# rwdavies/QUILT

Hardware: AMD Instinct MI355X
Metric: samples/sec on 2Mb region, K=50k haps, 1x coverage; dosage r2 vs CPU ref (higher is better)
Workload: dtype f64

## Files before the change

### quilt_amd/csrc/fullpass.hip

```cpp
#include "fullpass_dev.hpp"
#include "fullpass_testhook.h"
#include "pass_layout.hpp"

#include <algorithm>
#include <chrono>
#include <cmath>
#include <functional>
#include <memory>
#include <utility>

namespace {

template <typename TS>
__global__ __launch_bounds__(256) void k_emat(PassParams prm) {
    const int g = blockIdx.x, p = blockIdx.y, t = threadIdx.x;
    __shared__ double2 s_e[32];
    __shared__ double s_red[3][4];
    __shared__ int s_var;
    const int s = 32 * g;
    const int nLocal = min(32, prm.T - s);
    const double2 *gl = reinterpret_cast<const double2 *>(prm.gl) + (size_t)p * prm.T + s;
    if (t == 0) s_var = 0;
    __syncthreads();
    if (t < nLocal) {
// ... 638 lines not shown
    const int32_t *er = p.ent_read + p.ent_off[s], *eb = p.ent_bq + p.ent_off[s];
    const int32_t *H = p.H + p.pass_hoff[pi];
    double a = 1.0, b = 1.0;
    for (int i = sp[t]; i < sp[t + 1]; i++) {
        const int bq = eb[i];
        if (bq == 0 || H[er[i]] != lab) continue;
        const int ab = bq < 0 ? -bq : bq;
        a *= p.pR_tab[(bq > 0 ? 256 : 0) + ab];
        b *= p.pA_tab[(bq > 0 ? 256 : 0) + ab];
    }
    if (p.minGLValue > 0 && (a < p.minGLValue || b < p.minGLValue)) {
        if (a > b) { b = b / a; a = 1; if (b < p.minGLValue) b = p.minGLValue; }
        else       { a = a / b; b = 1; if (a < p.minGLValue) a = p.minGLValue; }
    }
    double2 *out = reinterpret_cast<double2 *>(p.gl) + (size_t)pi * p.T + t;
    *out = make_double2(a, b);
}

template <typename TS>
__global__ void k_unpermute(const TS *src, double *dst, int K, int Kq, int NT, int cols, size_t dst_ld) {
    constexpr int EPV = Vec<TS>::EPV, NV = 16 / EPV;
    const int col = blockIdx.y;
    const int k = blockIdx.x * blockDim.x + threadIdx.x;
    if (k >= K || col >= cols) return;
    const int chunk = k >> 4, e = k & 15;
    const int j = chunk / NT, t = chunk % NT;
    const size_t vec = alpha_vec_index<NV>(j, e / EPV, NT, t);
    dst[(size_t)col * dst_ld + k] = (double)src[(size_t)col * Kq + vec * EPV + (e % EPV)];
}

}

struct qa_panel::Scratch {
    qa::ABuf<double> gl, c, dosage, escale0, unperm, emin, emin_b1, spill, fw_add, fw_xs, gamma_col;
    qa::ABuf<char> emat, esp, alpha, gamma, beta, beta_thin, top_val, mg, gsp;
    qa::ABuf<int32_t> thin_col, flags, alpha_slot, top_cnt, top_idx;
    qa::DBuf<int32_t> todo;
    hipEvent_t ev[6] = {nullptr, nullptr, nullptr, nullptr, nullptr, nullptr};
    explicit Scratch(qa::Arena *a) {
        gl.arena = c.arena = dosage.arena = escale0.arena = unperm.arena = emin.arena = emin_b1.arena = spill.arena = fw_add.arena = fw_xs.arena = a;
        gamma_col.arena = a;
        emat.arena = esp.arena = alpha.arena = mg.arena = gsp.arena = gamma.arena = beta.arena = beta_thin.arena = top_val.arena = a;
        thin_col.arena = flags.arena = alpha_slot.arena = top_cnt.arena = top_idx.arena = a;
    }
    ~Scratch() {
        for (auto &e : ev) if (e) (void)hipEventDestroy(e);
    }
};

void qa::drop_pass_scratch(qa_panel *p) {
    delete p->scratch;
    p->scratch = nullptr;
}

qa_panel::~qa_panel() {
    delete scratch;
    if (gibbs_stream) (void)hipStreamDestroy(gibbs_stream);
    if (pass_stream) (void)hipStreamDestroy(pass_stream);
    if (stream) (void)hipStreamDestroy(stream);
}

namespace {

thread_local double g_timing[6] = {0, 0, 0, 0, 0, 0};

using qa::PassKind; using qa::KIND_F32; using qa::KIND_F64_RANK; using qa::KIND_F64_FULL; using qa::KIND_F64_DOS; using qa::KIND_F64_REF;
using qa::Geometry; using qa::PanelDims; using qa::PassLayout; using qa::Thin;
static_assert(qa::kLayoutMaxRow == kMaxRow, "pass_layout.hpp sizes emat / mg rows of kMaxRow");

struct KindInfo { const char *name; int pk_fwd, pk_bwd; };
constexpr KindInfo kKindInfo[qa::KIND_COUNT] = {
     {"fp32", qa::PK_FWD, qa::PK_BWD},
     {"fp64 ranking", qa::PK_FWD64, qa::PK_BWD64},
     {"generic fp64", qa::PK_FWD64G, qa::PK_BWD64G},
     {"fp64 dosage", qa::PK_FWD64D, qa::PK_BWD64D},
     {"reference-order validation", qa::PK_FWD64G, qa::PK_BWD64G},
};

constexpr int kNchList32[] = {1, 2, 3, 4, 5, 6, 7, 8, 10, 12};
constexpr int kNchList64[] = {1, 2, 4, 6, 8, 10, 12, 13, 14};
Geometry pick_geometry(int K, PassKind kind = KIND_F32) {
    const int chunks = (K + 15) / 16;
    if (kind == KIND_F64_RANK || kind == KIND_F64_DOS) {
        int nch = qa::fb64_chunks(K);
        if (kind == KIND_F64_DOS && nch && qa::fb64_dos_lds_bytes(K) > 160 * 1024) nch = 0;
        return {nch ? 512 : 0, nch, kind};
    }
    if (kind == KIND_F64_FULL || kind == KIND_F64_REF) {
        const int need = (K + 4095) / 4096;
        for (int nch : kNchList64) if (nch >= need) return {256, nch, kind};
        return {0, 0, kind};
    }
    auto fit = [&](int nch) -> int {
        int nt = (chunks + nch - 1) / nch;
        nt = std::max((nt + 63) / 64 * 64, 64);
        if (nt > 512) return 0;
        if (nch == 1 && chunks > 128) return 0;
        return nt;
    };
    for (int nch : kNchList32) if (int nt = fit(nch)) return {nt, nch, kind};
    return {0, 0, kind};
}


struct LastPlan { int64_t P = 0, per_pass = 0, fixed = 0, carved = 0, kind = 0; };
thread_local LastPlan g_last_plan;

PanelDims dims_of(const qa_panel *pn) { return {pn->K, pn->G, pn->T, pn->n_special, pn->n_sp_grids}; }

size_t plan_pass_bytes(const qa_panel *pn, const Geometry &geo, int32_t flag, const Thin &thin, int K_top, int top_cap = 64,
                       bool gamma_col = false) {
    return PassLayout(dims_of(pn), geo, qa::make_request(&flag, 1, thin, K_top, top_cap, gamma_col)).pass_bytes(qa::Arena::kCarveAlign);
}

int plan_chunk(qa_panel *pn, size_t per_pass, int remaining, size_t extra_fixed = 0) {
    const size_t fixed = (size_t)pn->G * 8 + ((size_t)2 << 20) + extra_fixed;
    g_last_plan.per_pass = (int64_t)per_pass;
    g_last_plan.fixed = (int64_t)fixed;
    const size_t budget = pn->plan_budget();
    long n = budget > fixed ? (long)((budget - fixed) / per_pass) : 0;
    n = std::max<long>(1, std::min<long>(n, remaining));
    static const int n_cu = [] {
        int dev = 0;
        hipDeviceProp_t prop;
        if (hipGetDevice(&dev) != hipSuccess || hipGetDeviceProperties(&prop, dev) != hipSuccess) return 256;
        return std::max(prop.multiProcessorCount, 1);
    }();
    if (n < remaining && n > n_cu) n = n / n_cu * n_cu;
    pn->require_scratch(fixed + (size_t)n * per_pass);
    pn->A().reset();
    return (int)n;
}

template <typename TS, int NCH, int MAXT, bool FULL>
void launch_fb(const PassParams &prm, int NT, hipStream_t s, hipEvent_t e_mid) {
    const size_t lds_f = 2 * kMaxRow * sizeof(TS) + 2 * 16 * 8;
    const size_t lds_b = lds_f + (FULL ? (size_t)2 * kMaxRow * kHistCopies * sizeof(typename Vec<TS>::Hist) : 0);
    hipLaunchKernelGGL((k_fwd<TS, NCH, MAXT>), dim3(prm.P), dim3(NT), lds_f, s, prm);
    QA_HIP(hipGetLastError());
// ... 142 lines not shown
std::vector<int32_t> plan_alpha_slots(const PassRun &r) {
    const int P = r.P, G = r.pn->G;
    std::vector<int32_t> slot((size_t)P * G, -1);
    for (int p = 0; p < P; p++) {
        int32_t *sl = slot.data() + (size_t)p * G;
        if ((r.h_flags[p] & 15) && r.geo.kind == KIND_F64_DOS) {
            for (int g = 0; g < G; g += 2) sl[g] = g / 2;
        } else if (r.h_flags[p] & 15) {
            for (int g = 0; g < G; g++) sl[g] = g;
        } else {
            int n = 0;
            for (int g = 0; g < G; g++) if (r.thin_col_h[g] >= 0) sl[g] = n++;
        }
    }
    return slot;
}

template <typename T>
void carve(qa::ABuf<T> &buf, const PassLayout &L, PassLayout::Buf b, int P) { buf.ensure(L.bytes(b, P) / sizeof(T)); }

void carve_scratch(qa_panel::Scratch &S, const PassLayout &L, int P, bool gl) {
    using B = PassLayout;
    if (gl) carve(S.gl, L, B::GL, P);
    carve(S.thin_col, L, B::THIN_COL, P);
    carve(S.flags, L, B::FLAGS, P);
    carve(S.alpha_slot, L, B::ALPHA_SLOT, P);
    carve(S.emat, L, B::EMAT, P);
    carve(S.escale0, L, B::ESCALE0, P);
    carve(S.emin, L, B::EMIN, P);
    carve(S.emin_b1, L, B::EMIN_B1, P);
    carve(S.esp, L, B::ESP, P);
    carve(S.gsp, L, B::GSP, P);
    carve(S.alpha, L, B::ALPHA, P);
    carve(S.c, L, B::C, P);
    carve(S.fw_add, L, B::FW_ADD, P);
    carve(S.fw_xs, L, B::FW_XS, P);
    carve(S.mg, L, B::MG, P);
    carve(S.dosage, L, B::DOSAGE, P);
    carve(S.gamma, L, B::GAMMA, P);
    carve(S.beta, L, B::BETA, P);
    carve(S.beta_thin, L, B::BETA_THIN, P);
    carve(S.gamma_col, L, B::GAMMA_COL, P);
    carve(S.top_cnt, L, B::TOP_CNT, P);
    carve(S.spill, L, B::SPILL, P);
    carve(S.top_idx, L, B::TOP_IDX, P);
    carve(S.top_val, L, B::TOP_VAL, P);
}

void fill_params(PassRun &r, int K_top, int normalize_emissions, int always_normalize, double norm_threshold) {
    const qa_panel *pn = r.pn;
    const auto &S = r.S;
    const PassLayout &L = r.L;
    const PassKind kind = r.geo.kind;
    PassParams &prm = r.prm;
    prm = PassParams{};
    prm.hm = pn->hm.p; prm.B = pn->B.p; prm.sp_off = pn->sp_off.p; prm.sp_k = pn->sp_k.p;
    prm.sp_word = pn->sp_word.p; prm.sp_gidx = pn->sp_gidx.p; prm.sp_chunk_at = pn->sp_chunk_at.p;
    prm.sigma = pn->sigma.p; prm.tm1 = pn->tm1.p; prm.IE = pn->ie_derived ? nullptr : pn->IE.p;
    prm.K = pn->K; prm.Kp = pn->Kp; prm.G = pn->G; prm.T = pn->T; prm.nMaxDH = pn->nMaxDH; prm.nrow = pn->nrow;
    prm.n_special = pn->n_special; prm.ref_error = pn->ref_error;
    prm.P = r.P; prm.gl = S.gl.p; prm.thin_col = S.thin_col.p; prm.n_thin = r.n_thin; prm.flags = S.flags.p;
    prm.normalize_emissions = normalize_emissions;
    prm.lazy = qa::lazy_kind(kind) ? 1 : 0; prm.always_normalize = always_normalize; prm.norm_threshold = norm_threshold;
    prm.grid0_left_to_right = pn->sum_order_grid0_ltr ? 1 : 0;
    prm.emin = S.emin.p; prm.emin_b1 = S.emin_b1.p; prm.esp_stride = (int)L.esp_stride;

    prm.spill = S.spill.p; prm.spill_pass_stride = L.spill_stride;
    prm.fw_add = S.fw_add.p; prm.fw_xs = S.fw_xs.p;
    prm.emat = S.emat.p; prm.esp = S.esp.p; prm.escale0 = S.escale0.p; prm.alpha = S.alpha.p; prm.alpha_slot = S.alpha_slot.p;
    prm.alpha_pass_stride = L.alpha_cols * L.alpha_col_elems; prm.Kq = (int)L.Kq; prm.alpha_col_elems = L.alpha_col_elems;
    prm.hist_unit = kind == KIND_F64_DOS ? 1.0 / 2251799813685248.0  : 1.0 / kHistScale64; prm.c = S.c.p; prm.mg = S.mg.p; prm.gsp = S.gsp.p;
    prm.gamma_out = S.gamma.p; prm.beta_out = S.beta.p;
    prm.gamma_col = S.gamma_col.p; prm.gamma_grid = r.out.gamma_col ? r.out.gamma_grid : -1;
    prm.K_top = r.any_top ? K_top : 0;
    prm.beta_thin = S.beta_thin.p;
    prm.fused_topk = r.fused ? 1 : 0;
    prm.top_cap = r.top_cap;
    prm.truncate_lists = r.out.truncate_lists ? 1 : 0;
    if (r.any_top) { prm.top_cnt = S.top_cnt.p; prm.top_idx = S.top_idx.p; prm.top_val = S.top_val.p; }
}

void choose_dosage_destination(PassRun &r) {
    const BatchOut &out = r.out;
    const int P = r.P, T = r.pn->T;
    bool direct = false;
    if (out.dosage && P > 0) {
        const size_t r0 = out.dosage_rows ? (size_t)out.dosage_rows[0] : 0;
        direct = true;
        for (int p = 0; p < P && direct; p++)
            direct = (r.h_flags[p] & 1) && (out.dosage_rows ? (size_t)out.dosage_rows[p] : (size_t)p) == r0 + (size_t)p;
        direct = direct && qa::pinned_registry().covers(out.dosage + r0 * T, sizeof(double) * (size_t)P * T);
        if (direct) r.prm.dosage = out.dosage + r0 * T;
    }
    if (!direct) r.prm.dosage = r.S.dosage.p;
    r.dosage_direct = direct;
}

void launch_passes(PassRun &r) {
    auto &S = r.S;
    const PassParams &prm = r.prm;
    const int P = r.P, G = r.pn->G;
// ... 294 lines not shown
    if (!out) return QA_ERR_INVALID;
    for (int i = 0; i < 3; i++) out[i] = g_timing[i];
    out[3] = g_timing[3] + g_timing[4];
    out[4] = g_timing[5];
    return QA_OK;
}

static int pack_lists(const std::vector<std::vector<std::pair<int32_t, double>>> &lists, int32_t *best_ptr,
                      int32_t *best_idx, double *best_val, int64_t best_cap) {
    if (!best_ptr) return QA_OK;
    int64_t total = 0;
    best_ptr[0] = 0;
    for (size_t i = 0; i < lists.size(); i++) {
        total += (int64_t)lists[i].size();
        best_ptr[i + 1] = (int32_t)total;
    }
    if (total > best_cap || !best_idx || !best_val) {
        qa::set_error("best-haps capacity %lld < needed %lld", (long long)best_cap, (long long)total);
        return QA_ERR_CAPACITY;
    }
    for (size_t i = 0; i < lists.size(); i++)
        for (size_t q = 0; q < lists[i].size(); q++) {
            best_idx[best_ptr[i] + q] = lists[i][q].first;
            best_val[best_ptr[i] + q] = (double)lists[i][q].second;
        }
    return QA_OK;
}

int qa_fullpass_last_plan(int64_t out[6]) {
    if (!out) return QA_ERR_INVALID;
    out[0] = g_last_plan.P; out[1] = g_last_plan.per_pass; out[2] = g_last_plan.fixed; out[3] = g_last_plan.carved;
    out[4] = PassLayout::N_BUF; out[5] = g_last_plan.kind;
    return QA_OK;
}

int qa_fullpass_launch_set(qa_panel_t *panel, int32_t n_pass, const double *gl, const int32_t *flags,
                           const int32_t *gammaSmall_cols_to_get, int32_t K_top_matches, int32_t always_normalize,
                           double *dosage, double *c, int32_t *best_ptr, int32_t *best_idx, double *best_val, int64_t best_cap) {
    if (!qa::device_ready()) return QA_ERR_NO_DEVICE;
    if (!panel || !gl || n_pass <= 0 || !flags || !gammaSmall_cols_to_get) {
        qa::set_error("qa_fullpass_launch_set: bad argument");
        return QA_ERR_INVALID;
    }
    int32_t any = 0;
    for (int i = 0; i < n_pass; i++) {
        if (flags[i] != 0 && flags[i] != 1) {
            qa::set_error("qa_fullpass_launch_set: flags must be 0 or 1");
            return QA_ERR_INVALID;
        }
        any |= flags[i];
    }
    return qa::guarded([&] {
        qa::GateHold hold;
        hold.acquire(panel->gate(), &panel->arena);
        QA_HIP(hipSetDevice(panel->device));
        const PassKind kind = dosage_kind(panel);
        const Thin thin = qa::count_thin(gammaSmall_cols_to_get, panel->G);
        const size_t retry = K_top_matches > 0 ? (size_t)n_pass * thin.n_thin * panel->K * 12 + 2 * qa::Arena::kCarveAlign : 0;
        if (plan_chunk(panel, plan_pass_bytes(panel, pick_geometry(panel->K, kind), any, thin, K_top_matches), n_pass, retry) < n_pass) {
            qa::set_error("qa_fullpass_launch_set: %d passes do not fit one launch set", n_pass);
            return (int)QA_ERR_CAPACITY;
        }
        std::vector<std::vector<std::pair<int32_t, double>>> lists;
        BatchOut out;
        out.dosage = dosage;
        out.c = c;
// ... 544 lines not shown
```

### quilt_amd/csrc/fullpass64.hip

```cpp
#include "fullpass_dev.hpp"

namespace {

constexpr int kNT = 512;
constexpr int kRowHaps = kNT * 16;
constexpr int kNStream = 8;

struct Geo64 { int NCH, NR, NL, n_last, NS; };

constexpr size_t kLdsFixed = 2 * kMaxRow * 8 + 2 * 16 * 8 + kNStream * 64 * 8 + 8 * kMaxTop * 8 + 64 + (size_t)kCandCap * 12;
constexpr size_t kLdsMax = 160 * 1024;

inline size_t lds_bytes(const Geo64 &g) { return kLdsFixed + (g.NL > 0 ? ((size_t)(g.NL - 1) * kNT + g.n_last) * 128 : 0); }
inline Geo64 geo64(int K) {
    Geo64 g{};
    g.NCH = (K + kRowHaps - 1) / kRowHaps;
    const int rem = K - (g.NCH - 1) * kRowHaps;
    g.n_last = ((rem + 15) / 16 + 63) / 64 * 64;
    g.NR = std::min(g.NCH, 4);
    g.NL = g.NCH - g.NR;
    if (lds_bytes(g) > kLdsMax) { g.NR = 5; g.NL = g.NCH - 5; }

    if (g.NCH > 7) {
        g.NS = g.NCH - 7;
// ... 293 lines not shown
                    for (int q = 0; q < 8; q++) {
                        double2 v = st[q * stride];
                        v.x *= xs; v.y *= xs;
                        st[q * stride] = v;
                    }
                }
            }
            if constexpr (SP) {
                for (int js = 0; js < NS; js++) {
                    double2 *st = spill_row(prm, p, js, tt);
#pragma unroll
                    for (int q = 0; q < 8; q++) {
                        double2 v = st[q * NT];
                        v.x *= xs; v.y *= xs;
                        st[q * NT] = v;
                    }
                }
            }
            cg = (g == 0) ? xs : cg / run_total;
            run_total = 1;
            running_min = 1;
        }
        prev_sum = run_total;
        if (tt == 0) {
            L.sc[SC_C * 64 + jl] = cg;
            if (prm.fw_add) {
                prm.fw_add[(size_t)p * G + g] = addend;
                prm.fw_xs[(size_t)p * G + g] = xs_of_grid;
            }
        }
        const int sl = (int)uniform(L.sc[SC_SLOT * 64 + jl]);
        if (sl >= 0) {
            double2 *dst = aout + (size_t)sl * col_vecs;
#pragma unroll
            for (int j = 0; j < NR; j++)
                if ((j * NT + tt) * 16 < K) store_chunk<double>(dst, a[j], j, NT, tt);
#pragma unroll
            for (int r = 0; r < NL; r++) {
                if ((r < NL - 1 || wave * 64 < n_last) && ((NR + r) * NT + tt) * 16 < K) {
                    const double2 *st = lds_row<NL>(L, r, tt);
                    const int stride = lds_stride<NL>(r, n_last);
#pragma unroll
                    for (int q = 0; q < 8; q++) dst[alpha_vec_index<8>(NR + r, q, NT, tt)] = st[q * stride];
                }
            }
            if constexpr (SP) {
                for (int js = 0; js < NS; js++) {
                    if (((NCH + js) * NT + tt) * 16 >= K) continue;
                    const double2 *st = spill_row(prm, p, js, tt);
#pragma unroll
                    for (int q = 0; q < 8; q++) dst[alpha_vec_index<8>(NCH + js, q, NT, tt)] = st[q * NT];
                }
            }
        }
    }
    __syncthreads();
    if (t < 64) {
        const int gb = (G - 1) & ~63;
        if (gb + lane < G) prm.c[(size_t)p * G + gb + lane] = L.sc[SC_C * 64 + lane];
    }
}

__device__ __forceinline__ void wave_top(double v, int Ktop, double *out, int lane) {
    for (int r = 0; r < Ktop; r++) {
        const double m = wave_max(v);
        const unsigned long long owners = __ballot(v == m);
        const int first = __ffsll((long long)owners) - 1;
        if (lane == first) v = -1.0;
        if (lane == 0) out[r] = m;
    }
}

template <int NR, int NL, bool SP = false>
__global__ __launch_bounds__(kNT) void k_bwd64(PassParams prm, int n_last) {
    constexpr int NCH = NR + NL, NT = kNT, nwaves = NT >> 6;
    const int NS = SP ? prm.Kq / kRowHaps - NCH : 0;
    extern __shared__ __attribute__((aligned(16))) char smem[];
    const Lds L(smem);
    const int p = blockIdx.x, t = threadIdx.x, lane = t & 63;
    const int wave = __builtin_amdgcn_readfirstlane(t >> 6);
    const uint32_t lds_etab = (uint32_t)(uintptr_t)(__attribute__((address_space(3))) char *)smem;
    const int K = prm.K, G = prm.G;
    const double *emat = static_cast<const double *>(prm.emat) + (size_t)p * G * kMaxRow;
    const double *esp = static_cast<const double *>(prm.esp) + (size_t)p * prm.esp_stride;
    const double *emin = prm.emin + (size_t)p * G;
    const size_t col_vecs = (size_t)prm.alpha_col_elems / 2;
    const size_t col_vecs_q = (size_t)prm.Kq / 2;
    const double *cvec = prm.c + (size_t)p * G;
    const int32_t *slot = prm.alpha_slot + (size_t)p * G;
    const double2 *ain = reinterpret_cast<const double2 *>(static_cast<const double *>(prm.alpha) + (size_t)p * prm.alpha_pass_stride);
    const double double_K = uniform((double)K);

    double b[NR][16];
    uint4 dh[NCH];
#pragma unroll
    for (int j = 0; j < NCH; j++) {
        const int k0 = (j * NT + t) * 16;
        if (j < NR) {
#pragma unroll
            for (int i = 0; i < 16; i++) b[j][i] = (k0 + i < K) ? 1.0 : 0.0;
        } else if (j - NR < NL - 1 || t < n_last) {
            double2 *st = lds_row<NL>(L, j - NR, t);
            const int stride = lds_stride<NL>(j - NR, n_last);
#pragma unroll
            for (int q = 0; q < 8; q++) st[q * stride] = make_double2(k0 + 2 * q < K ? 1.0 : 0.0, k0 + 2 * q + 1 < K ? 1.0 : 0.0);
        }
        dh[j] = *reinterpret_cast<const uint4 *>(prm.hm + (size_t)(G - 1) * prm.Kp + k0);
    }
    if constexpr (SP) {
        for (int js = 0; js < NS; js++) {
            double2 *st = spill_row(prm, p, js, t);
            const int k0 = ((NCH + js) * NT + t) * 16;
#pragma unroll
            for (int q = 0; q < 8; q++) st[q * NT] = make_double2(k0 + 2 * q < K ? 1.0 : 0.0, k0 + 2 * q + 1 < K ? 1.0 : 0.0);
        }
    }
    if (t < kMaxRow) L.etab[((G - 1) & 1) * kMaxRow + t] = emat[(size_t)(G - 1) * kMaxRow + t];
    if (t == 0) L.misc[0] = 0;
    __syncthreads();

    double val_prev = 0.0, x_prev = 1.0;
    double B_prev = 1, B_prev_star = uniform(double_K * cvec[G - 1] * 1.0);
    for (int g = G - 1; g >= 0; --g) {
        const int jl = g & 63;
        if (jl == 63 || g == G - 1) {
            __syncthreads();
            if (t < 64) {
                const int gb = g & ~63;
                const int gi = clampi(gb + lane, 0, G - 1), g1 = clampi(gb + lane + 1, 0, G - 1), gs = clampi(gb + lane, 0, G > 1 ? G - 2 : 0);
                L.sc[SC_SIG * 64 + lane] = G > 1 ? prm.sigma[gs] : 1.0;
                L.sc[SC_TM1 * 64 + lane] = G > 1 ? prm.tm1[gs] : 0.0;
                L.sc[SC_EMIN * 64 + lane] = g1 == 1 ? prm.emin_b1[p] : emin[g1];
                L.sc[SC_SPG * 64 + lane] = (double)prm.sp_gidx[g1];
                L.sc[SC_C * 64 + lane] = cvec[gi];
                L.sc[SC_SLOT * 64 + lane] = (double)slot[gi];
                L.sc[SC_TCOL * 64 + lane] = (double)prm.thin_col[gi];
            }
            __syncthreads();
        }
        const double c_g = uniform(L.sc[SC_C * 64 + jl]);
        double not_jump_prob = 1.0, val = 0.0;
        if (g < G - 1) {
            const int buf = (g + 1) & 1;
            const int tt = fresh_tid(wave);
            dma_table(emat, g, lds_etab, buf ^ 1, wave, tt & 63);
            const double jump_prob = uniform(L.sc[SC_TM1 * 64 + jl]) / double_K;
            not_jump_prob = uniform(L.sc[SC_SIG * 64 + jl]);
            const double *et = L.etab + buf * kMaxRow;
            const int sp_g = (int)uniform(L.sc[SC_SPG * 64 + jl]);
            const int32_t *sp_at = sp_g >= 0 ? prm.sp_chunk_at + (size_t)sp_g * (prm.Kq >> 4) : nullptr;
            const bool has_variant = uniform(L.sc[SC_EMIN * 64 + jl]) >= 0;
// ... 12 lines not shown
                dh[j] = reinterpret_cast<const uint4 *>(hm_next + j * kRowHaps)[tt];
            });
            if constexpr (SP) {
                const uint8_t *hm_e = prm.hm + (size_t)(g + 1) * prm.Kp;
                for (int js = 0; js < NS; js++) {
                    const int jg = NCH + js, k0 = (jg * NT + tt) * 16;
                    const uint4 d = reinterpret_cast<const uint4 *>(hm_e + (size_t)jg * kRowHaps)[tt];
                    psum += lds_chunk<true>(spill_row(prm, p, js, tt), NT, d, et, val_prev, x_prev, sp_at, esp, k0);
                }
            }
            const double sum_e_times_b = block_sum64<NCH>(psum, L.red + (g & 1) * 16, wave, lane, nwaves);
            if (has_variant) {
                val = uniform(jump_prob / not_jump_prob * sum_e_times_b);
                B_prev = sum_e_times_b;
            } else {
                val = uniform(jump_prob / not_jump_prob * B_prev_star);
                B_prev = B_prev_star;
            }
            B_prev_star = uniform(c_g * B_prev);
        }
        const int tcol = (int)uniform(L.sc[SC_TCOL * 64 + jl]);
        if (tcol >= 0 && prm.K_top > 0) {
            const int tp = fresh_tid(wave), lanep = tp & 63;
            const int sl = (int)uniform(L.sc[SC_SLOT * 64 + jl]);
            const double2 *av = ain + (size_t)sl * col_vecs;
            const int Ktop = prm.K_top;
            bool to_topk = !prm.fused_topk;
            auto beta_of = [&](auto jc, int q, const double2 *st, int stride) -> double2 {
                constexpr int j = decltype(jc)::value;
                if constexpr (j < NR) return make_double2(b[j][2 * q] + val, b[j][2 * q + 1] + val);
                else { const double2 u = st[q * stride]; return make_double2(u.x + val, u.y + val); }
            };
            if (prm.fused_topk) {
                double mx = 0.0;
                static_for<NCH>([&](auto jc) {
                    constexpr int j = decltype(jc)::value;
                    if constexpr (j > 0) return;
                    const int k0 = (j * NT + tp) * 16;
                    if (k0 >= K) return;
                    const double2 *st = j >= NR ? lds_row<NL>(L, j - NR, tp) : nullptr;
                    const int stride = j >= NR ? lds_stride<NL>(j - NR, n_last) : 0;
#pragma unroll
                    for (int q = 0; q < 8; q++) {
                        const double2 a2 = av[alpha_vec_index<8>(j, q, NT, tp)];
                        const double2 b2 = beta_of(jc, q, st, stride);
                        const double g0 = a2.x * b2.x, g1 = a2.y * b2.y;
                        mx = g0 > mx ? g0 : mx;
                        mx = g1 > mx ? g1 : mx;
                    }
                });
                wave_top(mx, Ktop, L.wtop + wave * kMaxTop, lanep);
                __syncthreads();
                double T0;
                {
                    double v = -1.0;
                    if (lanep < nwaves * Ktop) v = L.wtop[(lanep / Ktop) * kMaxTop + (lanep % Ktop)];
                    double m = 0;
                    for (int r = 0; r < Ktop; r++) {
                        m = wave_max(v);
                        const unsigned long long owners = __ballot(v == m);
                        const int first = __ffsll((long long)owners) - 1;
                        if (lanep == first) v = -1.0;
                    }
                    T0 = m > 0 ? m : 0.0;
                }
                static_for<NCH>([&](auto jc) {
                    constexpr int j = decltype(jc)::value;
                    const int k0 = (j * NT + tp) * 16;
                    if (k0 >= K) return;
                    const double2 *st = j >= NR ? lds_row<NL>(L, j - NR, tp) : nullptr;
                    const int stride = j >= NR ? lds_stride<NL>(j - NR, n_last) : 0;
#pragma unroll
                    for (int q = 0; q < 8; q++) {
                        const double2 a2 = av[alpha_vec_index<8>(j, q, NT, tp)];
                        const double2 b2 = beta_of(jc, q, st, stride);
                        const double gq[2] = {a2.x * b2.x, a2.y * b2.y};
#pragma unroll
                        for (int r = 0; r < 2; r++) {
                            if (gq[r] >= T0 && k0 + 2 * q + r < K) {
                                const int at = atomicAdd(&L.misc[0], 1);
                                if (at < kCandCap) { L.cand_v[at] = gq[r]; L.cand_k[at] = k0 + 2 * q + r; }
                            }
                        }
                    }
                });
                if constexpr (SP) {
                    for (int js = 0; js < NS; js++) {
                        const int k0 = ((NCH + js) * NT + tp) * 16;
                        if (k0 >= K) continue;
                        const double2 *st = spill_row(prm, p, js, tp);
#pragma unroll
                        for (int q = 0; q < 8; q++) {
                            const double2 a2 = av[alpha_vec_index<8>(NCH + js, q, NT, tp)];
                            const double2 u = st[q * NT];
                            const double gq[2] = {a2.x * (u.x + val), a2.y * (u.y + val)};
#pragma unroll
                            for (int r = 0; r < 2; r++) {
                                if (gq[r] >= T0 && k0 + 2 * q + r < K) {
                                    const int at = atomicAdd(&L.misc[0], 1);
// ... 18 lines not shown
                        const double v = c < n_c ? L.cand_v[c] : -1.0;
                        const int kk = c < n_c ? L.cand_k[c] : 0x7fffffff;
                        int rank = 0;
                        for (int m = 0; m < n_c; m++) {
                            const double vm = L.cand_v[m];
                            const int km = L.cand_k[m];
                            rank += (vm > v || (vm == v && km < kk)) ? 1 : 0;
                        }
                        if (c < n_c && rank == want - 1) *thr_slot = v;
                    }
                    __builtin_amdgcn_fence(__ATOMIC_RELEASE, "workgroup");
                    __builtin_amdgcn_wave_barrier();
                    __builtin_amdgcn_fence(__ATOMIC_ACQUIRE, "workgroup");
                    const double thr = want > 0 ? *thr_slot : 0.0;
                    int n_all = 0;
                    for (int c0 = 0; c0 < n_c; c0 += 64) {
                        const int c = c0 + lanep;
                        const double v = c < n_c ? L.cand_v[c] : -1.0;
                        const int kk = c < n_c ? L.cand_k[c] : 0x7fffffff;
                        const bool member = c < n_c && v >= thr;
                        n_all += __popcll(__ballot(member));
                        if (!__any(member)) continue;
                        int rank = 0;
                        for (int m = 0; m < n_c; m++) {
                            const double vm = L.cand_v[m];
                            const int km = L.cand_k[m];
                            rank += (vm > v || (vm == v && km < kk)) ? 1 : 0;
                        }
                        if (member && rank < prm.top_cap) { oi[rank] = kk; ov[rank] = v * not_jump_prob; }
                    }
                    if (lanep == 0) prm.top_cnt[(size_t)p * prm.n_thin + tcol] = n_all;
                }
                __syncthreads();
                if (tp == 0) L.misc[0] = 0;
            }
            if (to_topk && prm.beta_thin) {
                double2 *dst = reinterpret_cast<double2 *>(prm.beta_thin) + ((size_t)p * prm.n_thin + tcol) * col_vecs_q;
                static_for<NCH>([&](auto jc) {
                    constexpr int j = decltype(jc)::value;
                    const int k0 = (j * NT + tp) * 16;
                    if (k0 >= K) return;
                    const double2 *st = j >= NR ? lds_row<NL>(L, j - NR, tp) : nullptr;
                    const int stride = j >= NR ? lds_stride<NL>(j - NR, n_last) : 0;
#pragma unroll
                    for (int q = 0; q < 8; q++) dst[alpha_vec_index<8>(j, q, NT, tp)] = beta_of(jc, q, st, stride);
                });
                if constexpr (SP) {
                    for (int js = 0; js < NS; js++) {
                        if (((NCH + js) * NT + tp) * 16 >= K) continue;
                        const double2 *st = spill_row(prm, p, js, tp);
#pragma unroll
                        for (int q = 0; q < 8; q++) {
                            const double2 u = st[q * NT];
                            dst[alpha_vec_index<8>(NCH + js, q, NT, tp)] = make_double2(u.x + val, u.y + val);
                        }
                    }
                }
            }
        }
        val_prev = val;
        x_prev = uniform(c_g * not_jump_prob);
    }
}


constexpr int kHistCopiesD = 8;
constexpr int kNStreamD = 7;
// ... 309 lines not shown
            } else {
                val = uniform(jump_prob / not_jump_prob * B_prev_star);
                B_prev = B_prev_star;
            }
            B_prev_star = uniform(c_g * B_prev);
        }
        val_prev = val;
        x_prev = uniform(c_g * not_jump_prob);
        sig_prev = not_jump_prob;
    }
    {
        const int sp_g = prm.sp_gidx[0];
        const int32_t *sp_at = sp_g >= 0 ? prm.sp_chunk_at + (size_t)sp_g * (prm.Kq >> 4) : nullptr;
        process(std::false_type{}, 0, L.etab, sp_at, sp_g, val_prev, x_prev, sig_prev, false, 0.0, 1.0);
        asm volatile("s_waitcnt vmcnt(0) lgkmcnt(0)" ::: "memory");
        __builtin_amdgcn_s_barrier();
        asm volatile("" ::: "memory");
        fold(0);
    }
}

template <int NR, int NL, bool SP = false, bool GCOL = false>
void launch_dos(const PassParams &prm, const Geo64 &geo, hipStream_t s, hipEvent_t e_mid) {
    const size_t lds = lds_bytes(geo), lds_d = lds_bytes_d(geo);
    QA_HIP(hipFuncSetAttribute(reinterpret_cast<const void *>(k_fwd64<NR, NL, SP>), hipFuncAttributeMaxDynamicSharedMemorySize, (int)lds));
    hipLaunchKernelGGL((k_fwd64<NR, NL, SP>), dim3(prm.P), dim3(kNT), lds, s, prm, geo.n_last);
    QA_HIP(hipGetLastError());
    if (e_mid) QA_HIP(hipEventRecord(e_mid, s));
    QA_HIP(hipFuncSetAttribute(reinterpret_cast<const void *>(k_bwd64d<NR, NL, SP, GCOL>), hipFuncAttributeMaxDynamicSharedMemorySize, (int)lds_d));
    hipLaunchKernelGGL((k_bwd64d<NR, NL, SP, GCOL>), dim3(prm.P), dim3(kNT), lds_d, s, prm, geo.n_last);
    QA_HIP(hipGetLastError());
}

template <int NR, int NL, bool SP = false>
void launch(const PassParams &prm, const Geo64 &geo, hipStream_t s, hipEvent_t e_mid) {
    const size_t lds = lds_bytes(geo);
    QA_HIP(hipFuncSetAttribute(reinterpret_cast<const void *>(k_fwd64<NR, NL, SP>), hipFuncAttributeMaxDynamicSharedMemorySize, (int)lds));
    hipLaunchKernelGGL((k_fwd64<NR, NL, SP>), dim3(prm.P), dim3(kNT), lds, s, prm, geo.n_last);
    QA_HIP(hipGetLastError());
    if (e_mid) QA_HIP(hipEventRecord(e_mid, s));
    QA_HIP(hipFuncSetAttribute(reinterpret_cast<const void *>(k_bwd64<NR, NL, SP>), hipFuncAttributeMaxDynamicSharedMemorySize, (int)lds));
    hipLaunchKernelGGL((k_bwd64<NR, NL, SP>), dim3(prm.P), dim3(kNT), lds, s, prm, geo.n_last);
    QA_HIP(hipGetLastError());
}

template <bool GCOL>
void launch_dos_geo(const PassParams &prm, const Geo64 &geo, hipStream_t st, hipEvent_t e_mid) {
    if (geo.NS > 0) {
        launch_dos<5, 2, true, GCOL>(prm, geo, st, e_mid);
        return;
    }
    switch (geo.NR * 10 + geo.NL) {
#ifndef QA_FAST_BUILD
        case 10: launch_dos<1, 0, false, GCOL>(prm, geo, st, e_mid); break;
        case 20: launch_dos<2, 0, false, GCOL>(prm, geo, st, e_mid); break;
        case 30: launch_dos<3, 0, false, GCOL>(prm, geo, st, e_mid); break;
        case 40: launch_dos<4, 0, false, GCOL>(prm, geo, st, e_mid); break;
        case 41: launch_dos<4, 1, false, GCOL>(prm, geo, st, e_mid); break;
        case 42: launch_dos<4, 2, false, GCOL>(prm, geo, st, e_mid); break;
#endif
        case 52: launch_dos<5, 2, false, GCOL>(prm, geo, st, e_mid); break;
        case 43: launch_dos<4, 3, false, GCOL>(prm, geo, st, e_mid); break;
        default: throw std::runtime_error("fp64 geometry not built");
    }
}

}

namespace qa {

int fb64_chunks(int K) { const Geo64 g = geo64(K); return g.NCH + g.NS; }
int fb64_spill_rows(int K) { return geo64(K).NS; }
size_t fb64_lds_bytes(int K) { return lds_bytes(geo64(K)); }

size_t fb64_alpha_col_elems(int K) {
// ... 46 lines not shown
```

### quilt_amd/csrc/fullpass_dev.hpp

```cpp
#pragma once

#include "panel.hpp"

#include <type_traits>
#include <utility>

namespace {

constexpr int kMaxRow = 256;
constexpr int kHistCopies = 32;
constexpr float kHistScale = 2147483648.f;
constexpr double kHistScale64 = 4611686018427387904.0;
constexpr int kMaxTop = 8;
constexpr int kCandCap = 1024;

struct PassParams {
    const uint8_t *hm;
    const int32_t *B;
    const int32_t *sp_off;
    const int32_t *sp_k;
    const uint32_t *sp_word;
    const int32_t *sp_gidx;
    const int32_t *sp_chunk_at;
    const double *sigma;
// ... 13 lines not shown
    double norm_threshold;
    double *emin;
    double *emin_b1;
    void *emat;
    void *esp;
    int esp_stride;
    double *escale0;
    void *alpha;
    const int32_t *alpha_slot;
    size_t alpha_pass_stride;
    int Kq;
    size_t alpha_col_elems;
    double hist_unit;
    double *c;
    void *mg;
    void *gsp;
    void *gamma_out;
    void *beta_out;
    void *beta_thin;
    double *dosage;
    int K_top;
    int top_cap;
    int truncate_lists;
    int fused_topk;
    int32_t *top_cnt;
    int32_t *top_idx;
    void *top_val;
    const int32_t *topk_todo;
    double *fw_add, *fw_xs;
    double *spill;
    size_t spill_pass_stride;
    double *gamma_col;
    int gamma_grid;
};

__device__ __forceinline__ double word_emission(uint32_t w, const double2 *e, int nLocal) {
    double prob = 1.0;
    for (int b = 0; b < nLocal; b++) {
        const double2 v = e[b];
        prob *= ((w >> b) & 1u) ? v.y : v.x;
    }
    return prob;
}

__device__ __forceinline__ double wave_sum(double v) {
#pragma unroll
    for (int o = 32; o > 0; o >>= 1) v += __shfl_xor(v, o, 64);
    return v;
}
__device__ __forceinline__ double wave_min(double v) {
#pragma unroll
    for (int o = 32; o > 0; o >>= 1) v = fmin(v, __shfl_xor(v, o, 64));
    return v;
}
template <typename T>
__device__ __forceinline__ T wave_max(T v) {
#pragma unroll
    for (int o = 32; o > 0; o >>= 1) {
        const T w = __shfl_xor(v, o, 64);
        v = w > v ? w : v;
    }
    return v;
}

__device__ __noinline__ int special_lower_bound(const int32_t *sp_k, int lo, int hi, int k) {
    while (lo < hi) {
// ... 78 lines not shown
```

### quilt_amd/csrc/fullpass_testhook.h

```cpp
#ifndef QA_FULLPASS_TESTHOOK_H
#define QA_FULLPASS_TESTHOOK_H
#include <stdint.h>
#include "../../include/quilt_amd.h"
#ifdef __cplusplus
extern "C" {
#endif

int qa_fullpass_last_plan(int64_t out[6]);

int qa_fullpass_launch_set(qa_panel_t *panel, int32_t n_pass, const double *gl, const int32_t *flags,
                           const int32_t *gammaSmall_cols_to_get, int32_t K_top_matches, int32_t always_normalize,
                           double *dosage, double *c, int32_t *best_ptr, int32_t *best_idx, double *best_val, int64_t best_cap);

#ifdef __cplusplus
}
#endif
#endif
```

### quilt_amd/csrc/pass_layout.hpp

```cpp
#pragma once

#include <algorithm>
#include <cstddef>
#include <cstdint>

namespace qa {

int fb64_spill_rows(int K);
size_t fb64_alpha_col_elems(int K);
size_t fb_ref_state_doubles(int Kq);

enum PassKind { KIND_F32 = 0, KIND_F64_RANK = 1, KIND_F64_FULL = 2, KIND_F64_DOS = 3, KIND_F64_REF = 4, KIND_COUNT = 5 };
struct Geometry { int NT, NCH; PassKind kind; bool f64() const { return kind != KIND_F32; } };
inline bool lazy_kind(PassKind k) { return k == KIND_F64_RANK || k == KIND_F64_DOS || k == KIND_F64_REF; }

constexpr int kLayoutMaxRow = 256;

struct PanelDims { int K, G, T, n_special, n_sp_grids; };

struct Thin { int n_thin = 0, n_grids = 0; };
inline Thin count_thin(const int32_t *thin_col, int G) {
    Thin t;
    for (int g = 0; g < G; g++)
        if (thin_col[g] >= 0) { t.n_thin = std::max(t.n_thin, thin_col[g] + 1); t.n_grids++; }
    return t;
}

struct PassRequest {
    bool stores_all = false;
    bool gamma = false, beta = false, gamma_col = false;
    bool lists = false;
    Thin thin;
    int top_cap = 64;
};
inline PassRequest make_request(const int32_t *flags, int P, const Thin &thin, int K_top, int top_cap, bool gamma_col) {
    PassRequest r;
    for (int p = 0; p < P; p++) {
        r.stores_all |= (flags[p] & 15) != 0;
        r.gamma |= (flags[p] & 4) != 0;
        r.beta |= (flags[p] & 8) != 0;
    }
    r.lists = thin.n_thin > 0 && K_top > 0;
    r.thin = thin;
    r.top_cap = top_cap;
    r.gamma_col = gamma_col;
    return r;
}

struct PassLayout {
    enum Buf { GL, THIN_COL, FLAGS, ALPHA_SLOT, EMAT, ESCALE0, EMIN, EMIN_B1, ESP, GSP, ALPHA, C, FW_ADD, FW_XS, MG, DOSAGE, GAMMA,
               BETA, BETA_THIN, GAMMA_COL, TOP_CNT, SPILL, TOP_IDX, TOP_VAL, N_BUF };
    static constexpr size_t kAlphaSlack = (size_t)1 << 20;
    struct Entry { size_t elems = 0, elem_bytes = 1; };
    Entry e[N_BUF];
    size_t es = 4, Kq = 0, alpha_cols = 0, alpha_col_elems = 0, esp_stride = 0, spill_stride = 0;

    PassLayout(const PanelDims &d, const Geometry &geo, const PassRequest &r) {
        const PassKind kind = geo.kind;
        const size_t G = d.G, T = d.T, n_thin = r.thin.n_thin;
        es = geo.f64() ? 8 : 4;
        Kq = (size_t)geo.NT * geo.NCH * 16;
        alpha_cols = !r.stores_all ? (size_t)std::max(r.thin.n_grids, 1) : kind == KIND_F64_DOS ? (G + 1) / 2 : G;
        alpha_col_elems = kind == KIND_F64_DOS ? fb64_alpha_col_elems(d.K) : Kq;
        esp_stride = (size_t)d.n_special + (lazy_kind(kind) ? 16 * (size_t)d.n_sp_grids : 0) + 16;
        spill_stride = kind == KIND_F64_REF ? fb_ref_state_doubles((int)Kq)
                       : lazy_kind(kind) ? (size_t)fb64_spill_rows(d.K) * 8192 : 0;
        e[GL] = {T * 2, 8};
        e[THIN_COL] = {G, 4};
        e[FLAGS] = {1, 4};
        e[ALPHA_SLOT] = {G, 4};
        e[EMAT] = {G * kLayoutMaxRow, es};
        e[ESCALE0] = {1, 8};
        e[EMIN] = {G, 8};
        e[EMIN_B1] = {1, 8};
        e[ESP] = {esp_stride, es};
        e[GSP] = {(size_t)std::max(d.n_special, 1), es};
        e[ALPHA] = {alpha_cols * alpha_col_elems, es};
        e[C] = {G, 8};
        e[FW_ADD] = e[FW_XS] = {kind == KIND_F64_DOS ? G : 0, 8};
        e[MG] = {G * kLayoutMaxRow, es};
        e[DOSAGE] = {T, 8};
        e[GAMMA] = {r.gamma ? G * Kq : 0, es};
        e[BETA] = {r.beta ? G * Kq : 0, es};
        e[BETA_THIN] = {r.lists ? n_thin * Kq : 0, es};
        e[GAMMA_COL] = {r.gamma_col ? Kq : 0, 8};
        e[TOP_CNT] = {std::max<size_t>(n_thin, 1), 4};
        e[SPILL] = {spill_stride, 8};
        set_top_cap(r.lists ? r.top_cap : 0, n_thin);
    }
    void set_top_cap(int cap, size_t n_thin) {
        e[TOP_IDX] = {n_thin * (size_t)cap, 4};
        e[TOP_VAL] = {n_thin * (size_t)cap, es};
    }
    size_t bytes(Buf b, int P) const { return e[b].elems * e[b].elem_bytes * (b == THIN_COL ? 1 : (size_t)P) + (b == ALPHA ? kAlphaSlack : 0); }
    size_t pass_bytes(size_t align) const {
        size_t sum = 0;
        for (const Entry &x : e) sum += (x.elems * x.elem_bytes + align - 1) / align * align;
        return sum;
    }
};

}
```

Baseline: 37.02.

## Prune fused top-k backward scan using per-chunk alpha max bounds

```diff
diff --git a/quilt_amd/csrc/fullpass.hip b/quilt_amd/csrc/fullpass.hip
--- a/quilt_amd/csrc/fullpass.hip
+++ b/quilt_amd/csrc/fullpass.hip
@@ -694,14 +694,14 @@
 }
 
 struct qa_panel::Scratch {
-    qa::ABuf<double> gl, c, dosage, escale0, unperm, emin, emin_b1, spill, fw_add, fw_xs, gamma_col;
+    qa::ABuf<double> gl, c, dosage, escale0, unperm, emin, emin_b1, spill, fw_add, fw_xs, gamma_col, amax;
     qa::ABuf<char> emat, esp, alpha, gamma, beta, beta_thin, top_val, mg, gsp;
     qa::ABuf<int32_t> thin_col, flags, alpha_slot, top_cnt, top_idx;
     qa::DBuf<int32_t> todo;
     hipEvent_t ev[6] = {nullptr, nullptr, nullptr, nullptr, nullptr, nullptr};
     explicit Scratch(qa::Arena *a) {
         gl.arena = c.arena = dosage.arena = escale0.arena = unperm.arena = emin.arena = emin_b1.arena = spill.arena = fw_add.arena = fw_xs.arena = a;
-        gamma_col.arena = a;
+        gamma_col.arena = amax.arena = a;
         emat.arena = esp.arena = alpha.arena = mg.arena = gsp.arena = gamma.arena = beta.arena = beta_thin.arena = top_val.arena = a;
         thin_col.arena = flags.arena = alpha_slot.arena = top_cnt.arena = top_idx.arena = a;
     }
@@ -767,6 +767,9 @@
 
 struct LastPlan { int64_t P = 0, per_pass = 0, fixed = 0, carved = 0, kind = 0; };
 thread_local LastPlan g_last_plan;
+
+struct RankHook { int sparse_cap = -1; int32_t *path_cnt = nullptr; };
+RankHook g_rank_hook;
 
 PanelDims dims_of(const qa_panel *pn) { return {pn->K, pn->G, pn->T, pn->n_special, pn->n_sp_grids}; }
 
@@ -975,6 +978,7 @@
     carve(S.esp, L, B::ESP, P);
     carve(S.gsp, L, B::GSP, P);
     carve(S.alpha, L, B::ALPHA, P);
+    carve(S.amax, L, B::AMAX, P);
     carve(S.c, L, B::C, P);
     carve(S.fw_add, L, B::FW_ADD, P);
     carve(S.fw_xs, L, B::FW_XS, P);
@@ -1010,6 +1014,8 @@
 
     prm.spill = S.spill.p; prm.spill_pass_stride = L.spill_stride;
     prm.fw_add = S.fw_add.p; prm.fw_xs = S.fw_xs.p;
+    prm.amax = S.amax.p; prm.amax_pass_stride = L.alpha_cols * L.amax_col_elems;
+    prm.sparse_cap = g_rank_hook.sparse_cap; prm.path_cnt = g_rank_hook.path_cnt;
     prm.emat = S.emat.p; prm.esp = S.esp.p; prm.escale0 = S.escale0.p; prm.alpha = S.alpha.p; prm.alpha_slot = S.alpha_slot.p;
     prm.alpha_pass_stride = L.alpha_cols * L.alpha_col_elems; prm.Kq = (int)L.Kq; prm.alpha_col_elems = L.alpha_col_elems;
     prm.hist_unit = kind == KIND_F64_DOS ? 1.0 / 2251799813685248.0  : 1.0 / kHistScale64; prm.c = S.c.p; prm.mg = S.mg.p; prm.gsp = S.gsp.p;
@@ -1370,6 +1376,69 @@
     out[0] = g_last_plan.P; out[1] = g_last_plan.per_pass; out[2] = g_last_plan.fixed; out[3] = g_last_plan.carved;
     out[4] = PassLayout::N_BUF; out[5] = g_last_plan.kind;
     return QA_OK;
+}
+
+int qa_fullpass_rank_hook(int32_t sparse_cap, int32_t count, int64_t out[2]) {
+    g_rank_hook.sparse_cap = sparse_cap < 0 ? -1 : sparse_cap;
+    try {
+        if (out) {
+            out[0] = out[1] = 0;
+            if (g_rank_hook.path_cnt) {
+                int32_t h[2];
+                QA_HIP(hipMemcpy(h, g_rank_hook.path_cnt, sizeof(h), hipMemcpyDeviceToHost));
+                out[0] = h[0]; out[1] = h[1];
+            }
+        }
+        if (count && !g_rank_hook.path_cnt) QA_HIP(hipMalloc(reinterpret_cast<void **>(&g_rank_hook.path_cnt), 2 * sizeof(int32_t)));
+        if (count) QA_HIP(hipMemset(g_rank_hook.path_cnt, 0, 2 * sizeof(int32_t)));
+        if (!count && g_rank_hook.path_cnt) { QA_HIP(hipFree(g_rank_hook.path_cnt)); g_rank_hook.path_cnt = nullptr; }
+    } catch (const std::exception &e) {
+        qa::set_error("%s", e.what());
+        return QA_ERR_HIP;
+    }
+    return QA_OK;
+}
+
+int qa_fullpass_ranked_heads(qa_panel_t *panel, int32_t n_pass, const double *gl, const int32_t *gammaSmall_cols_to_get,
+                             int32_t K_top_matches, int32_t top_width, int32_t *top_idx, double *top_val, int32_t *top_cnt) {
+    if (!qa::device_ready()) return QA_ERR_NO_DEVICE;
+    if (!panel || !gl || n_pass <= 0 || !gammaSmall_cols_to_get || !top_idx || !top_val || !top_cnt || K_top_matches < 1 ||
+        top_width < K_top_matches || top_width > 64) {
+        qa::set_error("qa_fullpass_ranked_heads: bad argument");
+        return QA_ERR_INVALID;
+    }
+    return qa::guarded([&] {
+        qa::GateHold hold;
+        hold.acquire(panel->gate(), &panel->arena);
+        QA_HIP(hipSetDevice(panel->device));
+        const Thin thin = qa::count_thin(gammaSmall_cols_to_get, panel->G);
+        if (!panel->rank_fp64 || panel->sum_order_ref || thin.n_thin == 0 || pick_geometry(panel->K, KIND_F64_RANK).NT == 0) {
+            qa::set_error("qa_fullpass_ranked_heads: not a request the fp64 ranking kernels serve");
+            return (int)QA_ERR_UNSUPPORTED;
+        }
+        if (plan_chunk(panel, plan_pass_bytes(panel, pick_geometry(panel->K, KIND_F64_RANK), 0, thin, K_top_matches, top_width), n_pass) < n_pass) {
+            qa::set_error("qa_fullpass_ranked_heads: %d passes do not fit one launch set", n_pass);
+            return (int)QA_ERR_CAPACITY;
+        }
+        const std::vector<int32_t> flags(n_pass, 0);
+        std::vector<int32_t> fidx, cnt;
+        std::vector<double> fval;
+        BatchOut out;
+        out.flat_idx = &fidx; out.flat_val = &fval; out.true_counts = &cnt;
+        out.top_cap = top_width; out.order_by_value = true; out.truncate_lists = true;
+        const int status = run_passes(panel, n_pass, gl, flags.data(), gammaSmall_cols_to_get, K_top_matches, 1, out, KIND_F64_RANK);
+        if (status != QA_OK) return status;
+        const size_t n = (size_t)n_pass * thin.n_thin;
+        for (size_t i = 0; i < n; i++) {
+            top_cnt[i] = cnt[i];
+            for (int q = 0; q < top_width; q++) {
+                const bool have = q < std::min<int>(cnt[i], top_width);
+                top_idx[i * top_width + q] = have ? fidx[i * top_width + q] : -1;
+                top_val[i * top_width + q] = have ? fval[i * top_width + q] : 0.0;
+            }
+        }
+        return (int)QA_OK;
+    });
 }
 
 int qa_fullpass_launch_set(qa_panel_t *panel, int32_t n_pass, const double *gl, const int32_t *flags,
diff --git a/quilt_amd/csrc/fullpass64.hip b/quilt_amd/csrc/fullpass64.hip
--- a/quilt_amd/csrc/fullpass64.hip
+++ b/quilt_amd/csrc/fullpass64.hip
@@ -349,16 +349,32 @@
         const int sl = (int)uniform(L.sc[SC_SLOT * 64 + jl]);
         if (sl >= 0) {
             double2 *dst = aout + (size_t)sl * col_vecs;
+            double *amx = (!SP && prm.amax) ? prm.amax + (size_t)p * prm.amax_pass_stride + (size_t)sl * (prm.Kq >> 4) : nullptr;
 #pragma unroll
             for (int j = 0; j < NR; j++)
-                if ((j * NT + tt) * 16 < K) store_chunk<double>(dst, a[j], j, NT, tt);
+                if ((j * NT + tt) * 16 < K) {
+                    store_chunk<double>(dst, a[j], j, NT, tt);
+                    if (amx) {
+                        double m = a[j][0];
+#pragma unroll
+                        for (int i = 1; i < 16; i++) m = a[j][i] > m ? a[j][i] : m;
+                        amx[j * NT + tt] = m;
+                    }
+                }
 #pragma unroll
             for (int r = 0; r < NL; r++) {
                 if ((r < NL - 1 || wave * 64 < n_last) && ((NR + r) * NT + tt) * 16 < K) {
                     const double2 *st = lds_row<NL>(L, r, tt);
                     const int stride = lds_stride<NL>(r, n_last);
-#pragma unroll
-                    for (int q = 0; q < 8; q++) dst[alpha_vec_index<8>(NR + r, q, NT, tt)] = st[q * stride];
+                    double m = 0.0;
+#pragma unroll
+                    for (int q = 0; q < 8; q++) {
+                        const double2 u = st[q * stride];
+                        dst[alpha_vec_index<8>(NR + r, q, NT, tt)] = u;
+                        m = u.x > m ? u.x : m;
+                        m = u.y > m ? u.y : m;
+                    }
+                    if (amx) amx[(NR + r) * NT + tt] = m;
                 }
             }
             if constexpr (SP) {
@@ -389,7 +405,7 @@
 }
 
 template <int NR, int NL, bool SP = false>
-__global__ __launch_bounds__(kNT) void k_bwd64(PassParams prm, int n_last) {
+__global__ __launch_bounds__(kNT) void k_bwd64(PassParams prm, int n_last, int sparse_cap, int stage_cap) {
     constexpr int NCH = NR + NL, NT = kNT, nwaves = NT >> 6;
     const int NS = SP ? prm.Kq / kRowHaps - NCH : 0;
     extern __shared__ __attribute__((aligned(16))) char smem[];
@@ -433,7 +449,7 @@
         }
     }
     if (t < kMaxRow) L.etab[((G - 1) & 1) * kMaxRow + t] = emat[(size_t)(G - 1) * kMaxRow + t];
-    if (t == 0) L.misc[0] = 0;
+    if (t == 0) { L.misc[0] = 0; L.misc[1] = 0; }
     __syncthreads();
 
     double val_prev = 0.0, x_prev = 1.0;
@@ -512,6 +528,13 @@
                 else { const double2 u = st[q * stride]; return make_double2(u.x + val, u.y + val); }
             };
             if (prm.fused_topk) {
+                const bool sparse = !SP && sparse_cap > 0;
+                double am[NCH];
+                if (sparse) {
+                    const double *amc = prm.amax + (size_t)p * prm.amax_pass_stride + (size_t)sl * (prm.Kq >> 4);
+#pragma unroll
+                    for (int j = 1; j < NCH; j++) am[j] = (j * NT + tp) * 16 < K ? amc[j * NT + tp] : 0.0;
+                }
                 double mx = 0.0;
                 static_for<NCH>([&](auto jc) {
                     constexpr int j = decltype(jc)::value;
@@ -544,7 +567,84 @@
                     }
                     T0 = m > 0 ? m : 0.0;
                 }
-                static_for<NCH>([&](auto jc) {
+                bool dense = !sparse;
+                if (sparse) {
+                    double2 *stage = L.state + (NL > 0 ? ((size_t)(NL - 1) * NT + n_last) * 8 : 0);
+                    int *list = reinterpret_cast<int *>(stage + (size_t)stage_cap * 8);
+                    int slot_of[NCH];
+                    static_for<NCH>([&](auto jc) {
+                        constexpr int j = decltype(jc)::value;
+                        slot_of[j] = -1;
+                        if ((j * NT + tp) * 16 >= K) return;
+                        double bound = mx;
+                        if constexpr (j > 0) {
+                            double bm;
+                            if constexpr (j < NR) {
+                                bm = b[j][0];
+#pragma unroll
+                                for (int i = 1; i < 16; i++) bm = b[j][i] > bm ? b[j][i] : bm;
+                            } else {
+                                const double2 *st = lds_row<NL>(L, j - NR, tp);
+                                const int stride = lds_stride<NL>(j - NR, n_last);
+                                bm = 0.0;
+#pragma unroll
+                                for (int q = 0; q < 8; q++) {
+                                    const double2 u = st[q * stride];
+                                    bm = u.x > bm ? u.x : bm;
+                                    bm = u.y > bm ? u.y : bm;
+                                }
+                            }
+                            bound = am[j] * (bm + val);
+                        }
+                        if (bound >= T0) {
+                            const int at = atomicAdd(&L.misc[1], 1);
+                            slot_of[j] = at;
+                            if (at < sparse_cap) list[at] = j * NT + tp;
+                        }
+                    });
+                    __syncthreads();
+                    const int n_l = __builtin_amdgcn_readfirstlane(L.misc[1]);
+                    if (n_l > sparse_cap) {
+                        dense = true;
+                    } else {
+                        const uint32_t lds_stage = lds_etab + (uint32_t)(reinterpret_cast<char *>(stage) - smem);
+                        for (int base = 0; base < n_l; base += stage_cap) {
+                            const int n_b = n_l - base < stage_cap ? n_l - base : stage_cap;
+                            if (base > 0) __syncthreads();
+                            for (int m = wave; m * 8 < n_b; m += nwaves) {
+                                const int e = m * 8 + (lanep >> 3);
+                                const int id = list[base + (e < n_b ? e : n_b - 1)];
+                                dma16(av, (uint32_t)alpha_vec_index<8>(id / NT, lanep & 7, NT, id % NT) * 16u, lds_stage + (uint32_t)m * 1024u);
+                            }
+                            asm volatile("s_waitcnt vmcnt(0)" ::: "memory");
+                            __syncthreads();
+                            static_for<NCH>([&](auto jc) {
+                                constexpr int j = decltype(jc)::value;
+                                const int s_at = slot_of[j] - base;
+                                if (s_at < 0 || s_at >= n_b) return;
+                                const int k0 = (j * NT + tp) * 16;
+                                const double2 *sa = stage + (size_t)s_at * 8;
+                                const double2 *st = j >= NR ? lds_row<NL>(L, j - NR, tp) : nullptr;
+                                const int stride = j >= NR ? lds_stride<NL>(j - NR, n_last) : 0;
+#pragma unroll
+                                for (int q = 0; q < 8; q++) {
+                                    const double2 a2 = sa[q];
+                                    const double2 b2 = beta_of(jc, q, st, stride);
+                                    const double gq[2] = {a2.x * b2.x, a2.y * b2.y};
+#pragma unroll
+                                    for (int r = 0; r < 2; r++) {
+                                        if (gq[r] >= T0 && k0 + 2 * q + r < K) {
+                                            const int at = atomicAdd(&L.misc[0], 1);
+                                            if (at < kCandCap) { L.cand_v[at] = gq[r]; L.cand_k[at] = k0 + 2 * q + r; }
+                                        }
+                                    }
+                                }
+                            });
+                        }
+                    }
+                }
+                if (prm.path_cnt && tp == 0) atomicAdd(&prm.path_cnt[dense ? 1 : 0], 1);
+                if (dense) static_for<NCH>([&](auto jc) {
                     constexpr int j = decltype(jc)::value;
                     const int k0 = (j * NT + tp) * 16;
                     if (k0 >= K) return;
@@ -629,7 +729,7 @@
                     if (lanep == 0) prm.top_cnt[(size_t)p * prm.n_thin + tcol] = n_all;
                 }
                 __syncthreads();
-                if (tp == 0) L.misc[0] = 0;
+                if (tp == 0) { L.misc[0] = 0; L.misc[1] = 0; }
             }
             if (to_topk && prm.beta_thin) {
                 double2 *dst = reinterpret_cast<double2 *>(prm.beta_thin) + ((size_t)p * prm.n_thin + tcol) * col_vecs_q;
@@ -1005,15 +1105,32 @@
     QA_HIP(hipGetLastError());
 }
 
+struct SparseLds { int cap, stage_cap; size_t bytes; };
+inline SparseLds sparse_lds(const PassParams &prm, const Geo64 &geo, bool streamed) {
+    SparseLds s{0, 0, 0};
+    if (streamed || !prm.amax || !prm.fused_topk || prm.K_top <= 0 || prm.sparse_cap == 0) return s;
+    const size_t lds = lds_bytes(geo);
+    int cap = (((prm.K + 15) / 16 + 3) / 4 + 7) / 8 * 8;
+    if (prm.sparse_cap > 0) cap = std::min(cap, prm.sparse_cap);
+    const size_t list_bytes = (size_t)(cap + 3) / 4 * 16;
+    if (lds + list_bytes + 8 * 128 > kLdsMax) return s;
+    s.cap = cap;
+    s.stage_cap = (int)std::min<size_t>((kLdsMax - lds - list_bytes) / 128 / 8 * 8, (size_t)(cap + 7) / 8 * 8);
+    s.bytes = (size_t)s.stage_cap * 128 + list_bytes;
+    return s;
+}
+
 template <int NR, int NL, bool SP = false>
 void launch(const PassParams &prm, const Geo64 &geo, hipStream_t s, hipEvent_t e_mid) {
     const size_t lds = lds_bytes(geo);
+    const SparseLds sparse = sparse_lds(prm, geo, SP);
+    const size_t lds_b = lds + sparse.bytes;
     QA_HIP(hipFuncSetAttribute(reinterpret_cast<const void *>(k_fwd64<NR, NL, SP>), hipFuncAttributeMaxDynamicSharedMemorySize, (int)lds));
     hipLaunchKernelGGL((k_fwd64<NR, NL, SP>), dim3(prm.P), dim3(kNT), lds, s, prm, geo.n_last);
     QA_HIP(hipGetLastError());
     if (e_mid) QA_HIP(hipEventRecord(e_mid, s));
-    QA_HIP(hipFuncSetAttribute(reinterpret_cast<const void *>(k_bwd64<NR, NL, SP>), hipFuncAttributeMaxDynamicSharedMemorySize, (int)lds));
-    hipLaunchKernelGGL((k_bwd64<NR, NL, SP>), dim3(prm.P), dim3(kNT), lds, s, prm, geo.n_last);
+    QA_HIP(hipFuncSetAttribute(reinterpret_cast<const void *>(k_bwd64<NR, NL, SP>), hipFuncAttributeMaxDynamicSharedMemorySize, (int)lds_b));
+    hipLaunchKernelGGL((k_bwd64<NR, NL, SP>), dim3(prm.P), dim3(kNT), lds_b, s, prm, geo.n_last, sparse.cap, sparse.stage_cap);
     QA_HIP(hipGetLastError());
 }
 
diff --git a/quilt_amd/csrc/fullpass_dev.hpp b/quilt_amd/csrc/fullpass_dev.hpp
--- a/quilt_amd/csrc/fullpass_dev.hpp
+++ b/quilt_amd/csrc/fullpass_dev.hpp
@@ -69,6 +69,10 @@
     size_t spill_pass_stride;
     double *gamma_col;
     int gamma_grid;
+    double *amax;
+    size_t amax_pass_stride;
+    int sparse_cap;
+    int32_t *path_cnt;
 };
 
 __device__ __forceinline__ double word_emission(uint32_t w, const double2 *e, int nLocal) {
diff --git a/quilt_amd/csrc/fullpass_testhook.h b/quilt_amd/csrc/fullpass_testhook.h
--- a/quilt_amd/csrc/fullpass_testhook.h
+++ b/quilt_amd/csrc/fullpass_testhook.h
@@ -12,6 +12,11 @@
                            const int32_t *gammaSmall_cols_to_get, int32_t K_top_matches, int32_t always_normalize,
                            double *dosage, double *c, int32_t *best_ptr, int32_t *best_idx, double *best_val, int64_t best_cap);
 
+int qa_fullpass_ranked_heads(qa_panel_t *panel, int32_t n_pass, const double *gl, const int32_t *gammaSmall_cols_to_get,
+                             int32_t K_top_matches, int32_t top_width, int32_t *top_idx, double *top_val, int32_t *top_cnt);
+
+int qa_fullpass_rank_hook(int32_t sparse_cap, int32_t count, int64_t out[2]);
+
 #ifdef __cplusplus
 }
 #endif
diff --git a/quilt_amd/csrc/pass_layout.hpp b/quilt_amd/csrc/pass_layout.hpp
--- a/quilt_amd/csrc/pass_layout.hpp
+++ b/quilt_amd/csrc/pass_layout.hpp
@@ -48,12 +48,12 @@
 }
 
 struct PassLayout {
-    enum Buf { GL, THIN_COL, FLAGS, ALPHA_SLOT, EMAT, ESCALE0, EMIN, EMIN_B1, ESP, GSP, ALPHA, C, FW_ADD, FW_XS, MG, DOSAGE, GAMMA,
+    enum Buf { GL, THIN_COL, FLAGS, ALPHA_SLOT, EMAT, ESCALE0, EMIN, EMIN_B1, ESP, GSP, ALPHA, AMAX, C, FW_ADD, FW_XS, MG, DOSAGE, GAMMA,
                BETA, BETA_THIN, GAMMA_COL, TOP_CNT, SPILL, TOP_IDX, TOP_VAL, N_BUF };
     static constexpr size_t kAlphaSlack = (size_t)1 << 20;
     struct Entry { size_t elems = 0, elem_bytes = 1; };
     Entry e[N_BUF];
-    size_t es = 4, Kq = 0, alpha_cols = 0, alpha_col_elems = 0, esp_stride = 0, spill_stride = 0;
+    size_t es = 4, Kq = 0, alpha_cols = 0, alpha_col_elems = 0, amax_col_elems = 0, esp_stride = 0, spill_stride = 0;
 
     PassLayout(const PanelDims &d, const Geometry &geo, const PassRequest &r) {
         const PassKind kind = geo.kind;
@@ -76,6 +76,8 @@
         e[ESP] = {esp_stride, es};
         e[GSP] = {(size_t)std::max(d.n_special, 1), es};
         e[ALPHA] = {alpha_cols * alpha_col_elems, es};
+        amax_col_elems = kind == KIND_F64_RANK && r.lists && !r.stores_all ? Kq / 16 : 0;
+        e[AMAX] = {alpha_cols * amax_col_elems, 8};
         e[C] = {G, 8};
         e[FW_ADD] = e[FW_XS] = {kind == KIND_F64_DOS ? G : 0, 8};
         e[MG] = {G * kLayoutMaxRow, es};
```

Result: slower. 36.36 (-1.8%).
